# loicmagne/tinynerf

Hardware: AMD Instinct MI355X
Metric: ray-samples/sec (K-Planes training step: sampler + render fwd + bwd + Adam) (higher is better)
Workload: dtype f32 (f16x2-split products)

## Files before the change

include/tinynerf_hip.h:

```cpp
#ifndef TINYNERF_HIP_H
#define TINYNERF_HIP_H

#include <stdint.h>

#ifdef __cplusplus
extern "C" {
#endif

#define TN_ABI_VERSION 6

enum {
    TN_OK = 0,
    TN_E_NULL = -1,
    TN_E_SIZE = -2,
    TN_E_CONFIG = -3,
    TN_E_ALIGN = -4
};

const char *tn_last_error_string(void);
const char *tn_last_warning_string(void);
int tn_abi_version(void);

int tn_weights_fwd(const float *sigmas, const float *steps, const int32_t *info, float threshold,
                   float *weights, int64_t n_samples, int64_t n_rays, void *stream);
int tn_weights_fwd_gate(const float *sigmas, const float *steps, const int32_t *info, float threshold,
                        float *weights, float *gate, int64_t n_samples, int64_t n_rays, void *stream);
int tn_weights_bwd(const float *sigmas, const float *steps, const int32_t *info,
                   const float *weights, const float *grad_weights, float *grad_sigmas,
                   int64_t n_samples, int64_t n_rays, void *stream);

int tn_composite_fwd(const float *rgbs, const float *weights, const int32_t *info, const float *bg,
                     float *rendered, float *opacity, int64_t n_samples, int64_t n_rays, void *stream);
int tn_composite_bwd(const float *rgbs, const float *weights, const int32_t *info, const float *bg,
                     const float *grad_rendered, float *grad_rgbs, float *grad_weights,
                     int64_t n_samples, int64_t n_rays, void *stream);
int tn_ray_maps(const float *weights, const float *t_values, const int32_t *info, int64_t n_rays, float *opacity,
                float *depth, float *median_depth, void *stream);

int tn_occupancy_coarsen(const float *grid, int D, int H, int W, float *coarse, void *stream);
int tn_occupancy_query(const float *grid, int D, int H, int W, const float *coords, int64_t n,
                       float threshold, uint8_t *out, float *values, void *stream);
int tn_occupancy_slice_coords(int D, int H, int W, int slice, const float *jitter, uint64_t seed,
                              float *coords, void *stream);
int tn_occupancy_apply(float *grid_cells, const float *sigmas, int64_t n, float step_size,
                       float threshold, float decay, void *stream);
int tn_occupancy_stats(const float *grid, int64_t n, float threshold, double *stats, void *stream);

enum { TN_MARCH_AABB = 0, TN_MARCH_UNBOUNDED = 1 };
enum { TN_CONTRACT_AABB = 0, TN_CONTRACT_MIP360_INF = 1, TN_CONTRACT_MIP360_L2 = 2 };

typedef struct tn_sampler_desc {
    int32_t marcher;
    int32_t contraction;
    int32_t n_samples;
    int32_t grid_d, grid_h, grid_w;
    float aabb[6];
    float near, far;
    float step_size;
    float threshold;
    const float *t_table;
    const float *delta_table;
    const float *grid;
    const float *jitter;
    uint64_t seed;
    int32_t use_rng;
    int32_t reserved;
    const float *coarse;
} tn_sampler_desc;

int tn_march_rays(const tn_sampler_desc *desc, const float *rays_o, const float *rays_d, int64_t n_rays,
                  float *t_values, float *step_sizes, void *stream);
int tn_contract(const tn_sampler_desc *desc, const float *coords, int64_t n, float *coords_out,
                uint8_t *mask, void *stream);

int tn_sample_mask(const tn_sampler_desc *desc, const float *rays_o, const float *rays_d,
                   int64_t n_rays, uint64_t *maskbits, int32_t *counts, void *stream);
int tn_sample_scan(const int32_t *counts, int64_t n_rays, const int32_t *base_offset,
                   int32_t *info, int32_t *total, void *stream);
int tn_batch_plan(const int32_t *counts, int64_t n_rays, int32_t batch_size, int64_t target, int32_t *plan,
                  void *stream);
int tn_batch_plan_scan(const int32_t *counts, int64_t n_rays, int32_t batch_size, int64_t target, int32_t *plan,
                       int32_t *info, void *stream);
int tn_sample_pack(const tn_sampler_desc *desc, const float *rays_o, const float *rays_d,
                   int64_t n_rays, const uint64_t *maskbits, const int32_t *info,
                   const int32_t *base_offset, float *packed, int32_t *ray_ids, float *steps, int64_t capacity,
                   void *stream);
int tn_sample_pack_t(const tn_sampler_desc *desc, const float *rays_o, const float *rays_d,
                     int64_t n_rays, const uint64_t *maskbits, const int32_t *info,
                     const int32_t *base_offset, float *packed, int32_t *ray_ids, float *steps, float *t_values,
                     int64_t capacity, void *stream);

int tn_posenc_fwd(const float *x, int64_t n, int n_channels, const float *freqs, int n_freqs,
                  float *out, void *stream);

enum { TN_ACT_NONE = 0, TN_ACT_EXP_M1 = 1 , TN_ACT_SIGMOID = 2,
       TN_ACT_EXP = 3  };
enum { TN_ENC_NONE = 0,
       TN_ENC_POSENC = 1,
       TN_ENC_DIR_CAT = 2,
       TN_ENC_AUX_CAT = 3 };
#define TN_MLP_MAX_LAYERS 12
#define TN_MLP_ACCUM_GRAD_X 1
#define TN_MLP_STASHED 2
#define TN_MLP_CHAIN_ONLY 4
#define TN_MLP_WGRAD_ONLY 8
#define TN_MLP_GRAD_Y_ROWS 16

#define TN_MLP_BF16X3 32

#define TN_MLP_F16X2 64

#define TN_MLP_ROWS_ONLY 128
#define TN_MLP_X_FROM_ROWS 256

#define TN_MLP_SKIP_LAST 1024
#define TN_MLP_LAYERWISE 2048
#define TN_MLP_LEAN 512

typedef struct tn_mlp_desc {
    int32_t n_layers;
    int32_t in_dim;
    int32_t dims[TN_MLP_MAX_LAYERS + 1];
    int32_t encoding;
    int32_t n_freqs;
    int32_t out_activation;
    int32_t flags;
    const float *freqs;
    const float *weights[TN_MLP_MAX_LAYERS];
    const float *biases[TN_MLP_MAX_LAYERS];
    const int32_t *aux_index;
    int32_t aux_stride;
    int32_t reserved;
    const float *row_gate;
    const float *x_rows;
    float *grad_x_rows;
    int64_t x_rows_tile_stride;
    int64_t grad_x_rows_tile_stride;
    const void *grad_x_mask_rows;
    int64_t grad_x_mask_tile_stride;
} tn_mlp_desc;

#define TN_MERGE_MAX_HEADS 4
typedef struct tn_merge_head {
    const float *weight, *bias;
    int32_t rows, ld, col0, reserved;
    float *out_weight, *out_bias;
    const float *grad_merged_weight, *grad_merged_bias;
} tn_merge_head;
int tn_linear_merge_fwd(int32_t n_heads, const tn_merge_head *heads, const float *w_last, const float *b_last, int32_t F, void *stream);
int tn_linear_merge_bwd(int32_t n_heads, const tn_merge_head *heads, const float *w_last, const float *b_last, int32_t F,
                        float *grad_w_last, float *grad_b_last, void *stream);

int tn_linear_fwd(const float *x, const float *weight, const float *bias, int64_t n, int32_t in_features,
                  int32_t out_features, float *y, void *stream);
int tn_linear_bwd(const float *x, const float *weight, const float *grad_y, int64_t n, int32_t in_features,
                  int32_t out_features, float *grad_x, float *grad_weight, float *grad_bias, void *stream);

int tn_mlp_rows_view(const tn_mlp_desc *desc, int64_t n, int64_t *y_rows, int64_t *grad_y_rows, int64_t *tile_stride);
int tn_mlp_rows_view_hidden(const tn_mlp_desc *desc, int64_t n, int64_t *h_rows, int64_t *grad_h_rows, int64_t *mask_rows,
                            int64_t *tile_stride);

int tn_mlp_fwd(const tn_mlp_desc *desc, const float *x, const float *aux, int64_t n, float *y,
               float *pre_act, void *stream);
int64_t tn_mlp_fwd_workspace_bytes(const tn_mlp_desc *desc, int64_t n);
int tn_mlp_fwd_ws(const tn_mlp_desc *desc, const float *x, const float *aux, int64_t n, float *y, void *workspace,
                  int64_t workspace_bytes, void *stream);
int tn_mlp_fwd_stash(const tn_mlp_desc *desc, const float *x, const float *aux, int64_t n, float *y,
                     void *workspace, int64_t workspace_bytes, void *stream);
int tn_mlp_fwd_stash_pair(const tn_mlp_desc *desc, const tn_mlp_desc *partner, const float *x, const float *aux, int64_t n,
                          float *y, float *partner_y, void *workspace, int64_t workspace_bytes, void *partner_workspace,
                          int64_t partner_workspace_bytes, void *stream);
int tn_dir_encode(const float *dirs, int64_t n, const float *freqs, int n_freqs, float *out, int stride, void *stream);
int64_t tn_mlp_bwd_workspace_bytes(const tn_mlp_desc *desc, int64_t n);
int tn_mlp_bwd(const tn_mlp_desc *desc, const float *x, const float *aux, const float *grad_y,
               int64_t n, float *const *grad_weights, float *const *grad_biases, float *grad_x,
               void *workspace, int64_t workspace_bytes, void *stream);
int tn_mlp_bwd_pair(const tn_mlp_desc *desc, const tn_mlp_desc *partner, const float *x, const float *aux,
                    const float *grad_y, const float *partner_grad_y, int64_t n, float *const *grad_weights,
                    float *const *grad_biases, float *const *partner_grad_weights, float *const *partner_grad_biases,
                    float *grad_x, void *workspace, int64_t workspace_bytes, void *partner_workspace,
                    int64_t partner_workspace_bytes, void *stream);

int tn_mlp_lean_supported(const tn_mlp_desc *desc, const tn_mlp_desc *partner);

#define TN_KPLANES_MAX_SCALES 4
typedef struct tn_kplanes_desc {
    int32_t n_scales;
    int32_t channels;
    int32_t height[TN_KPLANES_MAX_SCALES];
    int32_t width[TN_KPLANES_MAX_SCALES];
    const float *planes[TN_KPLANES_MAX_SCALES][3];
} tn_kplanes_desc;

int tn_kplanes_fwd(const tn_kplanes_desc *desc, const float *x, int64_t x_stride, int64_t n,
                   float *feat, void *stream);
int tn_kplanes_bwd(const tn_kplanes_desc *desc, const float *x, int64_t x_stride, int64_t n,
                   const float *grad_feat, float *const (*grad_planes)[3], void *stream);

int tn_plane_reg_fwd(const float *plane, int H, int W, int C, double *sums, void *stream);
int tn_plane_reg_bwd(const float *plane, int H, int W, int C, float cy, float cx, float cl1,
// ... 90 lines not shown
```

tinynerf_amd/csrc/kplanes_device.h:

```cpp
#pragma once
#include "tn_common.h"

namespace tn {

typedef float f32x4k __attribute__((ext_vector_type(4)));

struct PlaneTaps {
    int off[4];
    float w[4];
    int cell;
};

__device__ __forceinline__ PlaneTaps plane_taps(float u, float v, int H, int W, int C) {
    PlaneTaps t;
    float u1 = u + 1.0f, v1 = v + 1.0f;
    asm volatile("" : "+v"(u1), "+v"(v1));
    float ix = (u1 * 0.5f) * (float)(W - 1);
    float iy = (v1 * 0.5f) * (float)(H - 1);
    asm volatile("" : "+v"(ix), "+v"(iy));
    const float x0f = floorf(ix), y0f = floorf(iy);
    const float fx = ix - x0f, fy = iy - y0f;
    const float gx = (x0f + 1.0f) - ix, gy = (y0f + 1.0f) - iy;
    t.w[0] = gx * gy; t.w[1] = fx * gy; t.w[2] = gx * fy; t.w[3] = fx * fy;
    const bool bx0 = x0f >= 0.0f && x0f < (float)W, bx1 = x0f + 1.0f >= 0.0f && x0f + 1.0f < (float)W;
    const bool by0 = y0f >= 0.0f && y0f < (float)H, by1 = y0f + 1.0f >= 0.0f && y0f + 1.0f < (float)H;
    const int x0 = bx0 ? (int)x0f : 0, x1 = bx1 ? (int)x0f + 1 : 0;
    const int y0 = by0 ? (int)y0f : 0, y1 = by1 ? (int)y0f + 1 : 0;
    t.off[0] = (bx0 && by0) ? (y0 * W + x0) * C : -1;
    t.off[1] = (bx1 && by0) ? (y0 * W + x1) * C : -1;
    t.off[2] = (bx0 && by1) ? (y1 * W + x0) * C : -1;
    t.off[3] = (bx1 && by1) ? (y1 * W + x1) * C : -1;
    const float cx = fminf(fmaxf(x0f, -2.0f), (float)W + 1.0f), cy = fminf(fmaxf(y0f, -2.0f), (float)H + 1.0f);
    t.cell = ((int)cy + 2) * (W + 4) + (int)cx + 2;
    return t;
}

template <int NV, int CS = 4>
__device__ __forceinline__ void plane_gather(const float *__restrict__ plane, const PlaneTaps &t, int c0, f32x4k (&out)[NV]) {
    f32x4k tex[4][NV];
    float w[4];
    const char *base = reinterpret_cast<const char *>(plane);
#pragma unroll
    for (int k = 0; k < 4; ++k) {
        const bool in = t.off[k] >= 0;
        unsigned boff = (unsigned)((in ? t.off[k] : 0) + c0) * 4u;
        asm volatile("" : "+v"(boff));
        w[k] = in ? t.w[k] : 0.0f;
#pragma unroll
        for (int v = 0; v < NV; ++v) tex[k][v] = *reinterpret_cast<const f32x4k *>(base + boff + (unsigned)(v * CS * 4));
    }
#pragma unroll
    for (int v = 0; v < NV; ++v) {
        f32x4k acc = tex[0][v] * w[0];
#pragma unroll
        for (int k = 1; k < 4; ++k)
#pragma unroll
            for (int e = 0; e < 4; ++e) acc[e] = __builtin_fmaf(tex[k][v][e], w[k], acc[e]);
        out[v] = acc;
    }
}

__device__ __forceinline__ void pair_uv(const float x[3], int p, float &u, float &v) {
    u = (p == 2) ? x[1] : x[0];
    v = (p == 0) ? x[1] : x[2];
}

}
```

tinynerf_amd/csrc/mlp.hip:

```cpp
#include "mlp_stage.h"
#include "mlp_f2_heads.h"
#include "kplanes_device.h"
#include <algorithm>

#ifdef TN_PHASE_TIMERS
__device__ unsigned long long tn_phase_cycles[16];
#define TN_PT_BEGIN unsigned long long pt_ = __builtin_amdgcn_s_memtime();
#define TN_PTG_BEGIN unsigned long long ptg_ = __builtin_amdgcn_s_memtime();
#define TN_PTG(k) { __builtin_amdgcn_sched_barrier(0); const unsigned long long n_ = __builtin_amdgcn_s_memtime(); if (lane == 0) atomicAdd(&tn_phase_cycles[k], n_ - ptg_); ptg_ = n_; }
#define TN_PT(k) { __builtin_amdgcn_sched_barrier(0); const unsigned long long n_ = __builtin_amdgcn_s_memtime(); if (lane == 0) atomicAdd(&tn_phase_cycles[k], n_ - pt_); pt_ = __builtin_amdgcn_s_memtime(); __builtin_amdgcn_sched_barrier(0); }
extern "C" int tn_debug_phase_cycles(unsigned long long *out, int reset) {
    hipMemcpyFromSymbol(out, HIP_SYMBOL(tn_phase_cycles), sizeof(unsigned long long) * 16);
    if (reset) { unsigned long long z[16] = {}; hipMemcpyToSymbol(HIP_SYMBOL(tn_phase_cycles), z, sizeof(z)); }
    return 0;
}
#else
#define TN_PT_BEGIN
#define TN_PT(k)
#define TN_PTG_BEGIN
#define TN_PTG(k)
#endif
namespace {

using tn::f32x16;
using tn::f32x4;
using namespace tn::mlp;

struct FwdPair { MlpArgs b; const float *aux; float *y; float *stash; };

struct KpFwd {
    int H[3], W[3];
    const float *planes[3][3];
    const float *coords;
    int64_t coord_stride;
    float *feat;
    int write_feat = 1;
};

#ifndef TN_F2_KP_WAVES
#define TN_F2_KP_WAVES 8
#endif
template <int H, bool WLDS, int WPB, bool STASH, bool PAIR = false, bool FAST = false, bool KP = false, bool F2 = false, int XB = 0, bool LEAN = false>
__global__ __launch_bounds__(WPB * 64) void mlp_fwd_kernel(MlpArgs a0, const float *__restrict__ x,
                                                           const float *__restrict__ aux0, int64_t n,
                                                           float *__restrict__ y0, float *__restrict__ pre_act0,
                                                           float *__restrict__ stash0, FwdPair pr, KpFwd kp = KpFwd())
{
    static_assert(!KP || (FAST && H == 64), "the fused gather feeds the plain-column first layer of the width-64 heads");
    static_assert(!F2 || (FAST && WLDS && H == 64), "f16x2 heads: plain-column first layer, weights in LDS, width 64");
    static_assert(!LEAN || (F2 && STASH && PAIR), "TN_MLP_LEAN: the paired f16x2 training forward");
    extern __shared__ __attribute__((aligned(16))) float lds[];
    constexpr int T = H / 32;
    if constexpr (F2) {
        stage_weights_f2(a0, lds);
        if constexpr (PAIR) stage_weights_f2(pr.b, lds + a0.lds_floats);
    } else if constexpr (WLDS) {
        stage_weights(a0, lds);
        if constexpr (PAIR) stage_weights(pr.b, lds + a0.lds_floats);
        __syncthreads();
    }
    const int lane = tn::lane_id(), j_ = lane & 31, h_ = lane >> 5;
    const int wave = __builtin_amdgcn_readfirstlane(threadIdx.x >> 6);
    const int64_t n_tiles = (n + 31) >> 5;

    for (int64_t tile = (int64_t)blockIdx.x * WPB + wave; tile < n_tiles; tile += (int64_t)gridDim.x * WPB) {
      constexpr bool PREF = F2 && (STASH || WPB <= 8);
      f32x4 avp[PREF ? 8 : 1];
      const bool pref_second = PAIR && pr.b.enc == TN_ENC_AUX_CAT;
      if constexpr (PREF) {
          const MlpArgs &ax = pref_second ? pr.b : a0;
          if (ax.enc == TN_ENC_AUX_CAT) {
              const float *auxp = pref_second ? pr.aux : aux0;
              const int64_t row = tile * 32 + j_;
              const int64_t rc = row < n ? row : 0;
              const float *arow = auxp + (int64_t)(ax.aux_index ? ax.aux_index[rc] : rc) * ax.aux_stride + 4 * h_;
              const int nga = (ax.K0_pad - ax.in_dim) >> 3;
#pragma unroll
              for (int g = 0; g < 8; ++g) avp[g] = *reinterpret_cast<const f32x4 *>(arow + 8 * (g < nga ? g : nga - 1));
          }
      }
      TN_PTG_BEGIN
      f32x4 fr[KP ? 12 : 1];
      if constexpr (KP) {
        int j = j_, h = h_;
        asm volatile("" : "+v"(j), "+v"(h));
        const int64_t row = tile * 32 + j;
        const bool valid = row < n;
        const float *cr = kp.coords + (valid ? row : 0) * kp.coord_stride;
        const float xs[3] = {cr[0], cr[1], cr[2]};
#pragma unroll
        for (int sc = 0; sc < 3; ++sc) {
            tn::f32x4k prod[4];
#pragma unroll
            for (int p = 0; p < 3; ++p) {
                float u, v;
                tn::pair_uv(xs, p, u, v);
                const tn::PlaneTaps t = tn::plane_taps(u, v, kp.H[sc], kp.W[sc], 32);
                tn::f32x4k val[4];
                tn::plane_gather<4, 8>(kp.planes[sc][p], t, 4 * h, val);
#pragma unroll
                for (int q = 0; q < 4; ++q) prod[q] = p == 0 ? val[q] : prod[q] * val[q];
                __builtin_amdgcn_sched_barrier(0);
            }
#pragma unroll
            for (int q = 0; q < 4; ++q) {
                fr[4 * sc + q] = f32x4{prod[q][0], prod[q][1], prod[q][2], prod[q][3]};
                if (valid && (STASH || !PAIR || kp.write_feat)) *reinterpret_cast<tn::f32x4k *>(kp.feat + row * 96 + 32 * sc + 8 * q + 4 * h) = prod[q];
            }
        }
      }
      u32x4h xbh[(F2 && KP) ? 6 : 1], xbl[(F2 && KP) ? 6 : 1];
      float inv_x = 1.0f;
      if constexpr (F2 && KP) {
          float m = 0.0f;
#pragma unroll
          for (int g = 0; g < 12; ++g)
#pragma unroll
              for (int u = 0; u < 4; ++u) m = fmaxf(m, fabsf(fr[g][u]));
          float s_x;
          f2_scales(f2_xmax(m), s_x, inv_x);
#pragma unroll
          for (int b = 0; b < 6; ++b) {
              const float v[8] = {fr[2 * b][0], fr[2 * b][1], fr[2 * b][2], fr[2 * b][3], fr[2 * b + 1][0], fr[2 * b + 1][1], fr[2 * b + 1][2], fr[2 * b + 1][3]};
              f2_split8(v, s_x, xbh[b], xbl[b]);
          }
      }
      TN_PTG(8)
      auto head2 = [&](const MlpArgs &a, const float *ldsw, const float *__restrict__ aux, float *__restrict__ y,
                       float *__restrict__ pre_act, float *__restrict__ stash, bool prefetched) {
        if constexpr (F2) {
        const int L = a.n_layers;
        int j = j_, h = h_;
        asm volatile("" : "+v"(j), "+v"(h));
        const int64_t row = tile * 32 + j;
        const bool valid = row < n;
        if constexpr (!STASH) {
            if (a.row_gate != nullptr) {
                const float gate = valid ? a.row_gate[row] : 0.0f;
                if (!__any(gate != 0.0f)) {
                    if (valid && h == 0) {
                        for (int o = 0; o < a.out_dim; ++o) {
                            y[row * a.out_dim + o] = 0.0f;
                            if (pre_act) pre_act[row * a.out_dim + o] = 0.0f;
                        }
                    }
                    return;
                }
            }
        }
        float *stH = nullptr, *stQ = nullptr;
        unsigned *stM = nullptr;
        if constexpr (STASH) {
            const int NH = L - 1;
            stH = stash + tile * (int64_t)(stash_rows(H, NH, 0) * 32);
            stQ = stH + stash_rows_w(H, NH, 0) * 32;
            stM = reinterpret_cast<unsigned *>(stQ + 4 * 32);
        }
        const float *scl = ldsw + a.f2_scale;
        TN_PT_BEGIN
        const _Float16 *W0 = reinterpret_cast<const _Float16 *>(ldsw + a.w_off[0]);
        const int plane0 = a.f2_plane[0], st0 = a.stride[0];
        const int nbx = a.in_dim >> 4;
        f32x16 acc[T];
#pragma unroll
        for (int ob = 0; ob < T; ++ob)
#pragma unroll
// ... 294 lines not shown
                    stM[(l * T + ob) * 64 + lane] = relu_bits(act[ob]);
                    store_rows(stH + l * H * 32, act[ob], ob, j, h);
                }
            }
        }
        const float *Wf = WLDS ? ldsw + a.w_off[L - 1] : a.W[L - 1];
        const float *Bf = WLDS ? ldsw + a.b_off[L - 1] : a.B[L - 1];
        const int sf = WLDS ? a.stride[L - 1] : H;
        const int out = a.out_dim;
        if (out <= 4) {
            float o4[4];
#pragma unroll
            for (int o = 0; o < 4; ++o) {
                o4[o] = 0.f;
                if (o < out) o4[o] = tn::small_out<H>(Wf + o * sf, Bf[o], act, h);
                if constexpr (STASH) { if (h == 0) stQ[o * 32 + j] = o4[o]; }
            }
            if (valid && h == 0) {
#pragma unroll
                for (int o = 0; o < 4; ++o)
                    if (o < out) {
                        if (pre_act) pre_act[row * out + o] = o4[o];
                        y[row * out + o] = tn::apply_act(o4[o], a.out_act);
                    }
            }
        } else {
            const int n_ob = (out + 31) >> 5;
            for (int ob = 0; ob < n_ob; ++ob) {
                f32x16 acc;
                if constexpr (WLDS) acc = tn::bias_tile(Bf, ob, h);
                else {
#pragma unroll
                    for (int r = 0; r < 16; ++r) {
                        const int f = 32 * ob + (r & 3) + 8 * (r >> 2) + 4 * h;
                        acc[r] = f < out ? Bf[f] : 0.f;
                    }
                }
                const int arow = 32 * ob + j;
#pragma unroll
                for (int kb = 0; kb < T; ++kb) {
#pragma unroll
                    for (int q = 0; q < 4; ++q) {
                        f32x4 w = {0.f, 0.f, 0.f, 0.f};
                        if (WLDS || arow < out) w = load_a4<WLDS>(Wf, arow, 32 * kb + 8 * q + 4 * h, H, sf);
#pragma unroll
                        for (int u = 0; u < 4; ++u) acc = tn::mfma32(w[u], act[kb][4 * q + u], acc);
                    }
                }
                tn::pin16(acc);
                if (valid) {
#pragma unroll
                    for (int q = 0; q < 4; ++q) {
                        const int f0 = 32 * ob + 8 * q + 4 * h;
                        if (f0 + 3 < out && (out & 3) == 0) {
                            f32x4 v;
#pragma unroll
                            for (int u = 0; u < 4; ++u) v[u] = acc[4 * q + u];
                            if (pre_act) *reinterpret_cast<f32x4 *>(pre_act + row * out + f0) = v;
#pragma unroll
                            for (int u = 0; u < 4; ++u) v[u] = tn::apply_act(v[u], a.out_act);
                            *reinterpret_cast<f32x4 *>(y + row * out + f0) = v;
                        } else {
#pragma unroll
                            for (int u = 0; u < 4; ++u)
                                if (f0 + u < out) {
                                    if (pre_act) pre_act[row * out + f0 + u] = acc[4 * q + u];
                                    y[row * out + f0 + u] = tn::apply_act(acc[4 * q + u], a.out_act);
                                }
                        }
                    }
                }
            }
        }
      };
      if constexpr (F2) {
          head2(a0, lds, aux0, y0, pre_act0, stash0, !pref_second);
          if constexpr (PAIR) head2(pr.b, lds + a0.lds_floats, pr.aux, pr.y, nullptr, pr.stash, pref_second);
          TN_PTG(9)
      } else {
          head(a0, lds, aux0, y0, pre_act0, stash0);
          if constexpr (PAIR) head(pr.b, lds + a0.lds_floats, pr.aux, pr.y, nullptr, pr.stash);
      }
    }
}

__global__ void posenc_kernel(const float *__restrict__ x, int64_t n, int C, const float *__restrict__ freqs, int F,
                              float *__restrict__ out)
{
    const int64_t e = (int64_t)blockIdx.x * blockDim.x + threadIdx.x;
    const int width = 2 * F * C;
    if (e >= n * width) return;
    const int64_t row = e / width;
    const int p = (int)(e - row * width);
    const int c = p / (2 * F);
    const int rem = p - c * 2 * F;
    const bool is_cos = rem >= F;
    const int f = is_cos ? rem - F : rem;
    const float ang = x[row * C + c] * (freqs ? freqs[f] : ldexpf(3.14159274101257324f, f));
    out[e] = is_cos ? cosf(ang) : sinf(ang);
}

using FwdKern = decltype(&mlp_fwd_kernel<32, false, 16, false>);

struct FwdPlan {
    MlpArgs a;
    FwdPair pr;
    KpFwd kp;
    FwdKern kern;
    int waves;
    size_t lds;
    int64_t blocks;
    const char *what;
};

bool plain_cols(const MlpArgs &m) { return m.enc == TN_ENC_AUX_CAT || (m.enc == TN_ENC_NONE && (m.in_dim & 3) == 0); }

bool f2_heads(const MlpArgs &a, const MlpArgs *b, bool kp) {
    if (!(f2_head_ok(a, 64) && (!b || f2_head_ok(*b, 64)) && (!kp || a.in_dim == 96))) return false;
    MlpArgs fa = a, fb = b ? *b : a;
    plan_f2(fa, 64); plan_f2(fb, 64);
    return ((size_t)fa.lds_floats + (b ? (size_t)fb.lds_floats : 0)) * 4 <= (size_t)LDS_LIMIT_BYTES;
}

template <int H>
int plan_fwd(FwdPlan &p, int64_t n, bool stash, bool pair, bool kp)
{
    MlpArgs &a = p.a;
    bool f2 = false;
    if constexpr (H == 64) f2 = f2_heads(a, pair ? &p.pr.b : nullptr, kp);
    if (f2) { plan_f2(a, H); if (pair) plan_f2(p.pr.b, H); }
    if (!pair) p.pr.b = a;
    p.lds = ((size_t)a.lds_floats + (pair ? (size_t)p.pr.b.lds_floats : 0)) * 4;
    const bool wlds = p.lds <= (size_t)LDS_LIMIT_BYTES && a.enc != -1;
    const bool fast = wlds && plain_cols(a) && (!pair || plain_cols(p.pr.b));
    constexpr int WPB = H <= 64 ? 16 : 4;
    p.waves = WPB; p.what = "mlp_fwd_kernel";
    if (a.x_from_rows && !(wlds && stash && H == 64 && !kp))
        return tn::fail(TN_E_CONFIG, "mlp forward: TN_MLP_X_FROM_ROWS is only read by tn_mlp_fwd_stash of a width-64 f16x2 head");
    if (!wlds) {
        if (stash) return tn::fail(TN_E_CONFIG, "tn_mlp_fwd_stash: weights must fit LDS");
        p.kern = mlp_fwd_kernel<H, false, WPB, false>; p.lds = 0; p.blocks = grid_blocks(n, WPB, 256 * 2);
        return TN_OK;
    }
    if constexpr (H == 64) {
        if (stash && kp) {
            if (!(fast && pair)) return tn::fail(TN_E_CONFIG, "tn_kplanes_mlp_fwd_pair: both heads must take the plain-column first layer");
            if (a.lean && !f2) return tn::fail(TN_E_CONFIG, "TN_MLP_LEAN needs the f16x2 heads (TN_MLP_F16X2)");
            p.kern = f2 ? (a.lean ? mlp_fwd_kernel<H, true, TN_F2_KP_WAVES, true, true, true, true, true, 0, true>
                                  : mlp_fwd_kernel<H, true, TN_F2_KP_WAVES, true, true, true, true, true>)
                        : mlp_fwd_kernel<H, true, 12, true, true, true, true>;
            p.waves = f2 ? TN_F2_KP_WAVES : 12; p.blocks = grid_blocks(n, p.waves, 256); p.what = "mlp_fwd_kernel(kplanes)";
            return TN_OK;
        }
        if (stash) {
            if (a.x_from_rows && !(f2 && !pair && a.x_rows != nullptr && (a.in_dim == 256 || a.in_dim == 128)))
                return tn::fail(TN_E_CONFIG, "tn_mlp_fwd_stash: TN_MLP_X_FROM_ROWS needs an f16x2 head with 128 or 256 inputs and x_rows");
            if (a.lean && !(f2 && pair)) return tn::fail(TN_E_CONFIG, "TN_MLP_LEAN needs the paired f16x2 heads (TN_MLP_F16X2, tn_mlp_fwd_stash_pair)");
            p.waves = 12;
            if (a.lean) p.kern = mlp_fwd_kernel<H, true, 12, true, true, true, false, true, 0, true>;
            else if (f2 && !pair && a.in_dim == 256) { p.kern = mlp_fwd_kernel<H, true, 8, true, false, true, false, true, 16>; p.waves = 8; }
            else if (f2 && !pair && a.in_dim == 128) p.kern = mlp_fwd_kernel<H, true, 12, true, false, true, false, true, 8>;
            else if (f2) p.kern = pair ? mlp_fwd_kernel<H, true, 12, true, true, true, false, true> : mlp_fwd_kernel<H, true, 12, true, false, true, false, true>;
            else if (fast) { p.kern = pair ? mlp_fwd_kernel<H, true, 16, true, true, true> : mlp_fwd_kernel<H, true, 16, true, false, true>; p.waves = 16; }
            else p.kern = pair ? mlp_fwd_kernel<H, true, 12, true, true, false> : mlp_fwd_kernel<H, true, 12, true, false, false>;
            p.blocks = grid_per_cu(n, p.waves, p.lds);
            return TN_OK;
        }
        if (kp) {
            if (!fast) return tn::fail(TN_E_CONFIG, "tn_kplanes_mlp_fwd: the head must take the plain-column first layer");
            p.kern = f2 ? (pair ? mlp_fwd_kernel<H, true, TN_F2_KP_WAVES, false, true, true, true, true>
                                : mlp_fwd_kernel<H, true, 12, false, false, true, true, true>)
                        : (pair ? mlp_fwd_kernel<H, true, 12, false, true, true, true> : mlp_fwd_kernel<H, true, 12, false, false, true, true>);
            p.waves = f2 && pair ? TN_F2_KP_WAVES : 12; p.blocks = grid_per_cu(n, p.waves, p.lds); p.what = "mlp_fwd_kernel(kplanes, inference)";
            return TN_OK;
        }
    } else if (stash) return tn::fail(TN_E_CONFIG, "tn_mlp_fwd_stash: the register-resident training forward is built for width 64");
    p.kern = fast ? mlp_fwd_kernel<H, true, WPB, false, false, true> : mlp_fwd_kernel<H, true, WPB, false, false, false>;
    if constexpr (H == 64) { if (f2) p.kern = mlp_fwd_kernel<H, true, WPB, false, false, true, false, true>; }
    p.blocks = grid_per_cu(n, WPB, p.lds);
    return TN_OK;
}

__global__ void dir_encode_kernel(const float *__restrict__ d, int64_t n, const float *__restrict__ freqs, int F, float *__restrict__ out, int stride)
{
    const int64_t e = (int64_t)blockIdx.x * blockDim.x + threadIdx.x;
    if (e >= n * stride) return;
    const int64_t row = e / stride;
    const int p = (int)(e - row * stride);
    const float dc[3] = {d[3 * row], d[3 * row + 1], d[3 * row + 2]};
    float v = 0.0f;
    if (p < 6 * F) v = tn::posenc_value(dc, p, F, freqs);
    else if (p < 6 * F + 3) v = dc[p - 6 * F];
    out[e] = v;
}

int fwd_common(const tn_mlp_desc *desc, const float *x, const float *aux, int64_t n, float *y, float *pre_act, float *stash,
               hipStream_t s, const FwdPair *pair = nullptr, const KpFwd *kp = nullptr)
{
    FwdPlan p;
    int H = 0;
    if (int rc = plan(desc, p.a, H)) return rc;
    const MlpArgs &a = p.a;
    TN_REQUIRE(n >= 0, TN_E_SIZE, "tn_mlp_fwd: negative n");
    if (n == 0) return TN_OK;
    TN_REQUIRE((x || kp) && y, TN_E_NULL, "tn_mlp_fwd: null pointer");
    TN_REQUIRE((a.enc != TN_ENC_DIR_CAT && a.enc != TN_ENC_AUX_CAT) || aux, TN_E_NULL, "tn_mlp_fwd: dir_cat / aux_cat need aux");
    TN_REQUIRE(((uintptr_t)x & 15) == 0 && ((uintptr_t)y & 15) == 0, TN_E_ALIGN, "tn_mlp_fwd: x / y must be 16-byte aligned");
    TN_REQUIRE(!kp || H == 64, TN_E_CONFIG, "tn_kplanes_mlp_fwd_pair: width-64 heads only");
    TN_REQUIRE(a.enc != TN_ENC_AUX_CAT || ((uintptr_t)aux & 15) == 0, TN_E_ALIGN, "tn_mlp_fwd: aux table must be 16-byte aligned");
    p.pr.aux = nullptr; p.pr.y = nullptr; p.pr.stash = nullptr;
    if (pair) p.pr = *pair;
    if (kp) p.kp = *kp;
    const int rc = H == 32 ? plan_fwd<32>(p, n, stash, pair, kp) : H == 64 ? plan_fwd<64>(p, n, stash, pair, kp)
                 : H == 128 ? plan_fwd<128>(p, n, stash, pair, kp) : plan_fwd<256>(p, n, stash, pair, kp);
    if (rc) return rc;
    return launch(p.kern, p.waves, p.lds, p.blocks, s, p.what, p.a, x, aux, n, y, pre_act, stash, p.pr, p.kp);
}

int partner_args(const tn_mlp_desc *partner, float *partner_y, void *partner_workspace, FwdPair &pr)
{
    int Hb = 0;
    if (int rc = plan(partner, pr.b, Hb)) return rc;
    pr.aux = nullptr; pr.y = partner_y; pr.stash = (float *)partner_workspace;
    return TN_OK;
}

}

extern "C" int tn_mlp_fwd(const tn_mlp_desc *desc, const float *x, const float *aux, int64_t n, float *y, float *pre_act,
                          void *stream)
{
    return fwd_common(desc, x, aux, n, y, pre_act, nullptr, (hipStream_t)stream);
}

extern "C" int64_t tn_mlp_bwd_workspace_bytes(const tn_mlp_desc *desc, int64_t n);

extern "C" int tn_mlp_fwd_stash_layers(const tn_mlp_desc *desc, const float *x, const float *aux, int64_t n, float *y, float *workspace,
                                       void *stream);

extern "C" int tn_mlp_fwd_stash(const tn_mlp_desc *desc, const float *x, const float *aux, int64_t n, float *y, void *workspace,
                                int64_t workspace_bytes, void *stream)
{
    TN_REQUIRE(desc, TN_E_NULL, "tn_mlp_fwd_stash: null descriptor");
    if (n <= 0) return n == 0 ? TN_OK : tn::fail(TN_E_SIZE, "tn_mlp_fwd_stash: negative n");
    const int64_t need = tn_mlp_bwd_workspace_bytes(desc, n);
    TN_REQUIRE(need > 0, TN_E_CONFIG, "tn_mlp_fwd_stash: this configuration's backward does not use a workspace");
    TN_REQUIRE(workspace && workspace_bytes >= need, TN_E_NULL, "tn_mlp_fwd_stash: workspace missing or too small");
    TN_REQUIRE(((uintptr_t)workspace & 15) == 0, TN_E_ALIGN, "tn_mlp_fwd_stash: workspace must be 16-byte aligned");
    if (!two_pass_supported(desc)) return tn_mlp_fwd_stash_layers(desc, x, aux, n, y, (float *)workspace, stream);
    return fwd_common(desc, x, aux, n, y, nullptr, (float *)workspace, (hipStream_t)stream);
}

extern "C" int tn_mlp_fwd_stash_pair(const tn_mlp_desc *desc, const tn_mlp_desc *partner, const float *x, const float *aux, int64_t n,
                                     float *y, float *partner_y, void *workspace, int64_t workspace_bytes, void *partner_workspace,
                                     int64_t partner_workspace_bytes, void *stream)
{
    TN_REQUIRE(desc && partner, TN_E_NULL, "tn_mlp_fwd_stash_pair: null descriptor");
    TN_REQUIRE(fwd_pair_shape_ok(desc, partner), TN_E_CONFIG,
               "tn_mlp_fwd_stash_pair: two width-64 heads (<= 5 layers, <= 4 outputs) on the same x; partner without encoding");
    if (n <= 0) return n == 0 ? TN_OK : tn::fail(TN_E_SIZE, "tn_mlp_fwd_stash_pair: negative n");
    const int64_t need_a = tn_mlp_bwd_workspace_bytes(desc, n), need_b = tn_mlp_bwd_workspace_bytes(partner, n);
    TN_REQUIRE(need_a > 0 && need_b > 0, TN_E_CONFIG, "tn_mlp_fwd_stash_pair: configuration not covered by the two-pass backward");
    TN_REQUIRE(workspace && workspace_bytes >= need_a && partner_workspace && partner_workspace_bytes >= need_b, TN_E_NULL,
               "tn_mlp_fwd_stash_pair: workspace missing or too small");
    TN_REQUIRE((((uintptr_t)workspace | (uintptr_t)partner_workspace | (uintptr_t)partner_y) & 15) == 0, TN_E_ALIGN,
               "tn_mlp_fwd_stash_pair: buffers must be 16-byte aligned");
    TN_REQUIRE(partner_y, TN_E_NULL, "tn_mlp_fwd_stash_pair: null pointer");
    FwdPair pr;
    if (int rc = partner_args(partner, partner_y, partner_workspace, pr)) return rc;
    return fwd_common(desc, x, aux, n, y, nullptr, (float *)workspace, (hipStream_t)stream, &pr);
}

extern "C" int tn_kplanes_mlp_fwd(const tn_kplanes_desc *kd, const float *coords, int64_t coord_stride, const tn_mlp_desc *desc, int64_t n,
                                  float *feat, float *y, void *stream)
{
    TN_REQUIRE(desc, TN_E_NULL, "tn_kplanes_mlp_fwd: null descriptor");
    TN_REQUIRE(desc->in_dim == 96 && desc->encoding == TN_ENC_NONE && desc->dims[1] == 64 && desc->row_gate == nullptr, TN_E_CONFIG,
               "tn_kplanes_mlp_fwd: an ungated width-64 head without encoding on the 96 features");
    if (n <= 0) return n == 0 ? TN_OK : tn::fail(TN_E_SIZE, "tn_kplanes_mlp_fwd: negative n");
    TN_REQUIRE(kd, TN_E_NULL, "tn_kplanes_mlp_fwd: null descriptor");
    TN_REQUIRE(kd->n_scales == 3 && kd->channels == 32, TN_E_CONFIG, "tn_kplanes_mlp_fwd: 3 scales x 32 channels (run.py:136)");
    TN_REQUIRE(coord_stride >= 3, TN_E_SIZE, "tn_kplanes_mlp_fwd: bad coordinate stride");
    TN_REQUIRE(coords && feat, TN_E_NULL, "tn_kplanes_mlp_fwd: null pointer");
    TN_REQUIRE(((uintptr_t)feat & 15) == 0, TN_E_ALIGN, "tn_kplanes_mlp_fwd: feat must be 16-byte aligned");
    KpFwd kp;
    if (int rc = kp_planes(kd, coords, coord_stride, kp)) return rc;
    kp.feat = feat;
    TN_REQUIRE(y && ((uintptr_t)y & 15) == 0, TN_E_ALIGN, "tn_kplanes_mlp_fwd: y must be a 16-byte aligned pointer");
    return fwd_common(desc, nullptr, nullptr, n, y, nullptr, nullptr, (hipStream_t)stream, nullptr, &kp);
}

extern "C" int tn_kplanes_mlp_fwd_pair(const tn_kplanes_desc *kd, const float *coords, int64_t coord_stride, const tn_mlp_desc *desc,
                                       const tn_mlp_desc *partner, const float *aux, int64_t n, float *feat, float *y, float *partner_y,
                                       void *workspace, int64_t workspace_bytes, void *partner_workspace, int64_t partner_workspace_bytes,
                                       void *stream)
{
    TN_REQUIRE(kd && desc && partner, TN_E_NULL, "tn_kplanes_mlp_fwd_pair: null descriptor");
    TN_REQUIRE(kd->n_scales == 3 && kd->channels == 32 && desc->in_dim == 96 && partner->in_dim == 96, TN_E_CONFIG,
               "tn_kplanes_mlp_fwd_pair: 3 scales x 32 channels feeding two heads with in_dim 96 (run.py:136-139)");
    TN_REQUIRE(coord_stride >= 3, TN_E_SIZE, "tn_kplanes_mlp_fwd_pair: bad coordinate stride");
    if (n <= 0) return n == 0 ? TN_OK : tn::fail(TN_E_SIZE, "tn_kplanes_mlp_fwd_pair: negative n");
    const bool inference = workspace == nullptr && partner_workspace == nullptr;
    TN_REQUIRE(coords && (feat || inference), TN_E_NULL, "tn_kplanes_mlp_fwd_pair: null pointer");
    TN_REQUIRE(((uintptr_t)feat & 15) == 0, TN_E_ALIGN, "tn_kplanes_mlp_fwd_pair: feat must be 16-byte aligned");
    TN_REQUIRE(!inference || ((uintptr_t)coords & 15) == 0, TN_E_ALIGN, "tn_kplanes_mlp_fwd_pair: coords must be 16-byte aligned");
    KpFwd kp;
    if (int rc = kp_planes(kd, coords, coord_stride, kp)) return rc;
    kp.feat = feat;
    if (inference) {
        kp.write_feat = 0;
// ... 40 lines not shown
```

Baseline: 343.6 million.

## Stream K-Planes bilinear taps through LDS with async global_load_lds software pipeline

```diff
diff --git a/include/tinynerf_hip.h b/include/tinynerf_hip.h
--- a/include/tinynerf_hip.h
+++ b/include/tinynerf_hip.h
@@ -19,6 +19,7 @@
 
 const char *tn_last_error_string(void);
 const char *tn_last_warning_string(void);
+int tn_debug_kp_gather_form(void);
 int tn_abi_version(void);
 
 int tn_weights_fwd(const float *sigmas, const float *steps, const int32_t *info, float threshold,
@@ -116,6 +117,7 @@
 #define TN_MLP_SKIP_LAST 1024
 #define TN_MLP_LAYERWISE 2048
 #define TN_MLP_LEAN 512
+#define TN_MLP_KP_GATHER_REGS 4096
 
 typedef struct tn_mlp_desc {
     int32_t n_layers;
diff --git a/tinynerf_amd/csrc/kplanes_device.h b/tinynerf_amd/csrc/kplanes_device.h
--- a/tinynerf_amd/csrc/kplanes_device.h
+++ b/tinynerf_amd/csrc/kplanes_device.h
@@ -60,6 +60,65 @@
     }
 }
 
+struct PlaneStage {
+    unsigned boff[4];
+    float w[4];
+};
+
+__device__ __forceinline__ PlaneStage plane_stage(const PlaneTaps &t, int c0) {
+    PlaneStage s;
+#pragma unroll
+    for (int k = 0; k < 4; ++k) {
+        const bool in = t.off[k] >= 0;
+        s.boff[k] = (unsigned)((in ? t.off[k] : 0) + c0) * 4u;
+        s.w[k] = in ? t.w[k] : 0.0f;
+    }
+    return s;
+}
+
+template <int V>
+__device__ __forceinline__ void plane_request(const float *plane, unsigned boff, unsigned area) {
+    unsigned keep;
+#ifdef TN_KP_GLDS_NO_IMM
+    asm volatile("s_mov_b32 %0, m0\n\ts_mov_b32 m0, %3\n\ts_nop 0\n\tglobal_load_lds_dwordx4 %1, %2\n\ts_mov_b32 m0, %0"
+                 : "=&s"(keep) : "v"(boff + (unsigned)(V * 32)), "s"(plane), "s"(area + (unsigned)(V * 1024)) : "memory");
+#else
+    asm volatile("s_mov_b32 %0, m0\n\ts_mov_b32 m0, %3\n\ts_nop 0\n\tglobal_load_lds_dwordx4 %1, %2 offset:%4\n\ts_mov_b32 m0, %0"
+                 : "=&s"(keep) : "v"(boff), "s"(plane), "s"(area + (unsigned)(V * 1024 - V * 32)), "n"(V * 32) : "memory");
+#endif
+}
+
+template <int V>
+__device__ __forceinline__ f32x4k plane_readback(unsigned lane_addr) {
+    f32x4k t;
+    asm volatile("s_waitcnt vmcnt(3)\n\tds_read_b128 %0, %1 offset:%2\n\ts_waitcnt lgkmcnt(0)" : "=&v"(t) : "v"(lane_addr), "n"(V * 1024) : "memory");
+    return t;
+}
+
+template <int K>
+__device__ __forceinline__ void plane_tap(const PlaneStage &s, unsigned area, unsigned lane_addr, const float *nplane, unsigned nboff, f32x4k (&acc)[4]) {
+    f32x4k tex[4];
+    tex[0] = plane_readback<0>(lane_addr); plane_request<0>(nplane, nboff, area);
+    tex[1] = plane_readback<1>(lane_addr); plane_request<1>(nplane, nboff, area);
+    tex[2] = plane_readback<2>(lane_addr); plane_request<2>(nplane, nboff, area);
+    tex[3] = plane_readback<3>(lane_addr); plane_request<3>(nplane, nboff, area);
+#pragma unroll
+    for (int v = 0; v < 4; ++v) {
+        if constexpr (K == 0) acc[v] = tex[v] * s.w[0];
+        else {
+#pragma unroll
+            for (int e = 0; e < 4; ++e) acc[v][e] = __builtin_fmaf(tex[v][e], s.w[K], acc[v][e]);
+        }
+    }
+}
+
+__device__ __forceinline__ void plane_first(const float *plane, unsigned boff, unsigned area) {
+    plane_request<0>(plane, boff, area); plane_request<1>(plane, boff, area);
+    plane_request<2>(plane, boff, area); plane_request<3>(plane, boff, area);
+}
+
+constexpr int KP_STAGE_BYTES = 4096;
+
 __device__ __forceinline__ void pair_uv(const float x[3], int p, float &u, float &v) {
     u = (p == 2) ? x[1] : x[0];
     v = (p == 0) ? x[1] : x[2];
diff --git a/tinynerf_amd/csrc/mlp.hip b/tinynerf_amd/csrc/mlp.hip
--- a/tinynerf_amd/csrc/mlp.hip
+++ b/tinynerf_amd/csrc/mlp.hip
@@ -35,12 +35,13 @@
     int64_t coord_stride;
     float *feat;
     int write_feat = 1;
+    unsigned stage = 0;
 };
 
 #ifndef TN_F2_KP_WAVES
 #define TN_F2_KP_WAVES 8
 #endif
-template <int H, bool WLDS, int WPB, bool STASH, bool PAIR = false, bool FAST = false, bool KP = false, bool F2 = false, int XB = 0, bool LEAN = false>
+template <int H, bool WLDS, int WPB, bool STASH, bool PAIR = false, bool FAST = false, bool KP = false, bool F2 = false, int XB = 0, bool LEAN = false, bool GL = false>
 __global__ __launch_bounds__(WPB * 64) void mlp_fwd_kernel(MlpArgs a0, const float *__restrict__ x,
                                                            const float *__restrict__ aux0, int64_t n,
                                                            float *__restrict__ y0, float *__restrict__ pre_act0,
@@ -49,6 +50,7 @@
     static_assert(!KP || (FAST && H == 64), "the fused gather feeds the plain-column first layer of the width-64 heads");
     static_assert(!F2 || (FAST && WLDS && H == 64), "f16x2 heads: plain-column first layer, weights in LDS, width 64");
     static_assert(!LEAN || (F2 && STASH && PAIR), "TN_MLP_LEAN: the paired f16x2 training forward");
+    static_assert(!GL || (KP && F2 && PAIR), "the LDS gather is built for the paired f16x2 forms");
     extern __shared__ __attribute__((aligned(16))) float lds[];
     constexpr int T = H / 32;
     if constexpr (F2) {
@@ -63,10 +65,33 @@
     const int wave = __builtin_amdgcn_readfirstlane(threadIdx.x >> 6);
     const int64_t n_tiles = (n + 31) >> 5;
 
+    unsigned area = 0, lane_addr = 0;
+    float xa[3] = {0.f, 0.f, 0.f};
+    auto coords_of = [&](int64_t t, float (&xo)[3]) {
+        const int64_t row = t * 32 + j_;
+        const float *cr = kp.coords + (row < n ? row : 0) * kp.coord_stride;
+        xo[0] = cr[0]; xo[1] = cr[1]; xo[2] = cr[2];
+    };
+    auto stage_of = [&](const float (&xo)[3], int sc, int p) {
+        float u, v;
+        tn::pair_uv(xo, p, u, v);
+        return tn::plane_stage(tn::plane_taps(u, v, kp.H[sc], kp.W[sc], 32), 4 * h_);
+    };
+    if constexpr (GL) {
+        area = (unsigned)reinterpret_cast<uintptr_t>((__attribute__((address_space(3))) void *)lds) + kp.stage + (unsigned)wave * (unsigned)tn::KP_STAGE_BYTES;
+        lane_addr = area + 16u * (unsigned)lane;
+        coords_of((int64_t)blockIdx.x * WPB + wave, xa);
+        tn::plane_first(kp.planes[0][0], stage_of(xa, 0, 0).boff[0], area);
+    }
+
     for (int64_t tile = (int64_t)blockIdx.x * WPB + wave; tile < n_tiles; tile += (int64_t)gridDim.x * WPB) {
       constexpr bool PREF = F2 && (STASH || WPB <= 8);
       f32x4 avp[PREF ? 8 : 1];
       const bool pref_second = PAIR && pr.b.enc == TN_ENC_AUX_CAT;
+      const float *avrow = nullptr;
+      int avn = 0;
+      float xn[3] = {0.f, 0.f, 0.f};
+      if constexpr (GL) coords_of(tile + (int64_t)gridDim.x * WPB, xn);
       if constexpr (PREF) {
           const MlpArgs &ax = pref_second ? pr.b : a0;
           if (ax.enc == TN_ENC_AUX_CAT) {
@@ -75,13 +100,60 @@
               const int64_t rc = row < n ? row : 0;
               const float *arow = auxp + (int64_t)(ax.aux_index ? ax.aux_index[rc] : rc) * ax.aux_stride + 4 * h_;
               const int nga = (ax.K0_pad - ax.in_dim) >> 3;
-#pragma unroll
-              for (int g = 0; g < 8; ++g) avp[g] = *reinterpret_cast<const f32x4 *>(arow + 8 * (g < nga ? g : nga - 1));
+              avrow = arow; avn = nga;
+              if constexpr (!GL) {
+#pragma unroll
+                  for (int g = 0; g < 8; ++g) avp[g] = *reinterpret_cast<const f32x4 *>(arow + 8 * (g < nga ? g : nga - 1));
+              }
           }
       }
       TN_PTG_BEGIN
       f32x4 fr[KP ? 12 : 1];
-      if constexpr (KP) {
+      if constexpr (KP && GL) {
+        uint64_t avaddr = reinterpret_cast<uint64_t>(avrow);
+        asm volatile("" : "+v"(xn[0]), "+v"(xn[1]), "+v"(xn[2]), "+v"(avaddr));
+        const global_char *avg = reinterpret_cast<const global_char *>(avaddr);
+        int j = j_, h = h_;
+        asm volatile("" : "+v"(j), "+v"(h));
+        const int64_t row = tile * 32 + j;
+        const bool valid = row < n;
+        tn::PlaneStage st = stage_of(xa, 0, 0);
+#pragma unroll
+        for (int sc = 0; sc < 3; ++sc) {
+            tn::f32x4k prod[4];
+#pragma unroll
+            for (int p = 0; p < 3; ++p) {
+                const int q9 = 3 * sc + p;
+                const int nsc = q9 == 8 ? 0 : (q9 + 1) / 3, np = q9 == 8 ? 0 : (q9 + 1) % 3;
+                const tn::PlaneStage nst = q9 == 8 ? stage_of(xn, 0, 0) : stage_of(xa, nsc, np);
+                tn::f32x4k val[4];
+                tn::plane_tap<0>(st, area, lane_addr, kp.planes[sc][p], st.boff[1], val);
+                if constexpr (PREF) {
+                    if (q9 == 0 && avrow != nullptr) {
+#pragma unroll
+                        for (int g = 0; g < 8; ++g) avp[g] = *reinterpret_cast<const __attribute__((address_space(1))) f32x4 *>(avg + 32 * (g < avn ? g : avn - 1));
+                    }
+                }
+                tn::plane_tap<1>(st, area, lane_addr, kp.planes[sc][p], st.boff[2], val);
+                tn::plane_tap<2>(st, area, lane_addr, kp.planes[sc][p], st.boff[3], val);
+                if constexpr (PREF) {
+                    if (q9 == 8) asm volatile("" : "+v"(avp[0]), "+v"(avp[1]), "+v"(avp[2]), "+v"(avp[3]), "+v"(avp[4]), "+v"(avp[5]), "+v"(avp[6]), "+v"(avp[7]));
+                }
+                tn::plane_tap<3>(st, area, lane_addr, kp.planes[nsc][np], nst.boff[0], val);
+#pragma unroll
+                for (int q = 0; q < 4; ++q) prod[q] = p == 0 ? val[q] : prod[q] * val[q];
+                st = nst;
+            }
+#pragma unroll
+            for (int q = 0; q < 4; ++q) fr[4 * sc + q] = f32x4{prod[q][0], prod[q][1], prod[q][2], prod[q][3]};
+        }
+        if (valid && (STASH || kp.write_feat)) {
+#pragma unroll
+            for (int g = 0; g < 12; ++g)
+                *reinterpret_cast<tn::f32x4k *>(kp.feat + row * 96 + 32 * (g >> 2) + 8 * (g & 3) + 4 * h) = tn::f32x4k{fr[g][0], fr[g][1], fr[g][2], fr[g][3]};
+        }
+        xa[0] = xn[0]; xa[1] = xn[1]; xa[2] = xn[2];
+      } else if constexpr (KP) {
         int j = j_, h = h_;
         asm volatile("" : "+v"(j), "+v"(h));
         const int64_t row = tile * 32 + j;
@@ -542,6 +614,7 @@
           if constexpr (PAIR) head(pr.b, lds + a0.lds_floats, pr.aux, pr.y, nullptr, pr.stash);
       }
     }
+    if constexpr (GL) asm volatile("s_waitcnt vmcnt(0)" ::: "memory");
 }
 
 __global__ void posenc_kernel(const float *__restrict__ x, int64_t n, int C, const float *__restrict__ freqs, int F,
@@ -571,7 +644,18 @@
     size_t lds;
     int64_t blocks;
     const char *what;
+    bool kp_regs = false;
 };
+
+thread_local int g_kp_gather_form = 0;
+
+bool plan_kp_lds(FwdPlan &p, int waves) {
+    const size_t stage = (size_t)waves * tn::KP_STAGE_BYTES;
+    const bool fits = !p.kp_regs && p.lds + stage <= (size_t)LDS_LIMIT_BYTES;
+    if (fits) { p.kp.stage = (unsigned)p.lds; p.lds += stage; }
+    g_kp_gather_form = fits ? 2 : 1;
+    return fits;
+}
 
 bool plain_cols(const MlpArgs &m) { return m.enc == TN_ENC_AUX_CAT || (m.enc == TN_ENC_NONE && (m.in_dim & 3) == 0); }
 
@@ -609,6 +693,10 @@
             p.kern = f2 ? (a.lean ? mlp_fwd_kernel<H, true, TN_F2_KP_WAVES, true, true, true, true, true, 0, true>
                                   : mlp_fwd_kernel<H, true, TN_F2_KP_WAVES, true, true, true, true, true>)
                         : mlp_fwd_kernel<H, true, 12, true, true, true, true>;
+            g_kp_gather_form = 1;
+            if (f2 && plan_kp_lds(p, TN_F2_KP_WAVES))
+                p.kern = a.lean ? mlp_fwd_kernel<H, true, TN_F2_KP_WAVES, true, true, true, true, true, 0, true, true>
+                                : mlp_fwd_kernel<H, true, TN_F2_KP_WAVES, true, true, true, true, true, 0, false, true>;
             p.waves = f2 ? TN_F2_KP_WAVES : 12; p.blocks = grid_blocks(n, p.waves, 256); p.what = "mlp_fwd_kernel(kplanes)";
             return TN_OK;
         }
@@ -631,6 +719,8 @@
             p.kern = f2 ? (pair ? mlp_fwd_kernel<H, true, TN_F2_KP_WAVES, false, true, true, true, true>
                                 : mlp_fwd_kernel<H, true, 12, false, false, true, true, true>)
                         : (pair ? mlp_fwd_kernel<H, true, 12, false, true, true, true> : mlp_fwd_kernel<H, true, 12, false, false, true, true>);
+            g_kp_gather_form = 1;
+            if (f2 && pair && plan_kp_lds(p, TN_F2_KP_WAVES)) p.kern = mlp_fwd_kernel<H, true, TN_F2_KP_WAVES, false, true, true, true, true, 0, false, true>;
             p.waves = f2 && pair ? TN_F2_KP_WAVES : 12; p.blocks = grid_per_cu(n, p.waves, p.lds); p.what = "mlp_fwd_kernel(kplanes, inference)";
             return TN_OK;
         }
@@ -671,6 +761,7 @@
     p.pr.aux = nullptr; p.pr.y = nullptr; p.pr.stash = nullptr;
     if (pair) p.pr = *pair;
     if (kp) p.kp = *kp;
+    p.kp_regs = (desc->flags & TN_MLP_KP_GATHER_REGS) != 0;
     const int rc = H == 32 ? plan_fwd<32>(p, n, stash, pair, kp) : H == 64 ? plan_fwd<64>(p, n, stash, pair, kp)
                  : H == 128 ? plan_fwd<128>(p, n, stash, pair, kp) : plan_fwd<256>(p, n, stash, pair, kp);
     if (rc) return rc;
@@ -686,6 +777,8 @@
 }
 
 }
+
+extern "C" int tn_debug_kp_gather_form(void) { return g_kp_gather_form; }
 
 extern "C" int tn_mlp_fwd(const tn_mlp_desc *desc, const float *x, const float *aux, int64_t n, float *y, float *pre_act,
                           void *stream)
```

Result: no change. 342.4 million, median of 4 (-0.4%).
